# d8ahazard/AudioLab

Hardware: AMD Instinct MI355X
Metric: stems*realtime-factor (44.1kHz stereo) (higher is better)
Workload: dtype bf16; 1 GPU; MDX-Net UVR 4-stem (4x TFC-TDF U-Net L=11 g=48 dim_f=3072 dim_t=256 n_fft=6144), 300 s 44.1 kHz stereo in total, margin chunker, windows/launch=52; stems=4

## Files before the change

audiolab_amd/csrc/tdfnet.hip:

```cpp
#include "mma.h"
#include <alsep_gfx950_asm.h>

#include <map>
#include <type_traits>

namespace {

constexpr int kThreads = 256;

template <typename T> struct Vec16;
template <> struct Vec16<float> { static constexpr int N = 4; };
template <> struct Vec16<bf16_t> { static constexpr int N = 8; };
__device__ __forceinline__ void store_vec(float* p, const float* y) { *reinterpret_cast<float4*>(p) = make_float4(y[0], y[1], y[2], y[3]); }
__device__ __forceinline__ void store_vec(bf16_t* p, const float* y) {
    bf16x8 q;
#pragma unroll
    for (int e = 0; e < 8; ++e) q[e] = (bf16_t)y[e];
    *reinterpret_cast<bf16x8*>(p) = q;
}
__device__ __forceinline__ void load_vec(const float* p, float* x) {
    const float4 q = *reinterpret_cast<const float4*>(p);
    x[0] = q.x; x[1] = q.y; x[2] = q.z; x[3] = q.w;
}
__device__ __forceinline__ void load_vec(const bf16_t* p, float* x) {
// ... 2109 lines not shown
template <int C_, int OCC>
__global__ void __launch_bounds__(kThreads, OCC)
ds_split_stream_kernel(const bf16_t* __restrict__ X, bf16_t* __restrict__ Y, const bf16_t* __restrict__ Wf,
                       const float* __restrict__ scale, const float* __restrict__ shift, int64_t npix, int Tp, int Fp) {
    typedef DsSplitCfg<C_> D;
    const int tid = threadIdx.x, lane = tid & 63, wave = tid >> 6;
    const int l15 = lane & 15, lq = lane >> 4;
    bf16_t* stg = reinterpret_cast<bf16_t*>(alsep_smem);
    bf16x8 wf[D::MTW][D::KS];
#pragma unroll
    for (int j = 0; j < D::MTW; ++j) {
        const int mt = wave + 4 * j;
#pragma unroll
        for (int ks = 0; ks < D::KS; ++ks)
            wf[j][ks] = mt < D::MT ? *reinterpret_cast<const bf16x8*>(Wf + ((size_t)(mt * D::KS + ks) * 64 + lane) * 8) : bf16x8{};
    }
    const int64_t ntile = npix / 64;
    for (int64_t tile = blockIdx.x; tile < ntile; tile += gridDim.x) {
        const int64_t p0 = tile * 64;
        const int64_t fp0 = p0 % Fp, tp = (p0 / Fp) % Tp, bb = p0 / ((int64_t)Fp * Tp);
        const bf16_t* xrow = X + ((bb * 2 * Tp + 2 * tp) * (2 * (int64_t)Fp) + 2 * fp0) * D::C;
        f32x4 acc[D::MTW][4];
#pragma unroll
        for (int j = 0; j < D::MTW; ++j)
#pragma unroll
            for (int ni = 0; ni < 4; ++ni) acc[j][ni] = f32x4{0.f, 0.f, 0.f, 0.f};
#pragma unroll
        for (int ks = 0; ks < D::KS; ++ks) {
            const int k = ks * 32 + lq * 8;
            const int dy = k / (2 * D::C), rem = k % (2 * D::C);
            bf16x8 xf[4];
#pragma unroll
            for (int ni = 0; ni < 4; ++ni)
                xf[ni] = *reinterpret_cast<const bf16x8*>(xrow + (int64_t)dy * (2 * (int64_t)Fp * D::C) + (int64_t)(ni * 16 + l15) * (2 * D::C) + rem);
#pragma unroll
            for (int j = 0; j < D::MTW; ++j)
                if (wave + 4 * j < D::MT) {
#pragma unroll
                    for (int ni = 0; ni < 4; ++ni) mma_step(acc[j][ni], wf[j][ks], xf[ni]);
                }
        }
#pragma unroll
        for (int j = 0; j < D::MTW; ++j) {
            const int mt = wave + 4 * j;
            if (mt < D::MT) {
                const f32x4 scv = *reinterpret_cast<const f32x4*>(scale + mt * 16 + 4 * lq);
                const f32x4 shv = *reinterpret_cast<const f32x4*>(shift + mt * 16 + 4 * lq);
#pragma unroll
                for (int ni = 0; ni < 4; ++ni) {
                    float y[4];
#pragma unroll
                    for (int r = 0; r < 4; ++r) y[r] = fmaxf(fmaf(acc[j][ni][r], scv[r], shv[r]), 0.f);
                    store4(stg + (ni * 16 + l15) * D::MS + mt * 16 + 4 * lq, y);
                }
            }
        }
        __syncthreads();
        bf16_t* yrow = Y + p0 * D::M;
        for (int it = tid; it < 64 * D::M / 8; it += kThreads)
            *reinterpret_cast<vec16*>(yrow + (size_t)it * 8) = lds_read16_align8(stg + (it / (D::M / 8)) * D::MS + (it % (D::M / 8)) * 8);
        __syncthreads();
    }
}

template <int CIN, int C2_, int NI_> struct UsCfg {
    static constexpr int C = CIN, C2 = C2_, NI = NI_, PX = 16 * NI_, MT = C2_ / 16, KS = (CIN + 31) / 32;
    static constexpr int PS = C2_ + 4;
    static constexpr size_t lds_bytes = 2 * (size_t)(2 * PX) * PS * sizeof(float);
    static_assert(C2_ % 16 == 0 && CIN % 8 == 0 && (2 * 2 * PX * (C2_ / 8)) % kThreads == 0, "us stream geometry");
};
template <int CIN, int C2_, int NI_, int OCC = 1>
__global__ void __launch_bounds__(kThreads, OCC)
us_stream_kernel(const bf16_t* __restrict__ X, bf16_t* __restrict__ Y, const bf16_t* __restrict__ Wf,
                 const float* __restrict__ scale, const float* __restrict__ shift, const bf16_t* __restrict__ skip,
                 int64_t npix, int Tp, int Fp) {
    typedef UsCfg<CIN, C2_, NI_> U;
    const int tid = threadIdx.x, lane = tid & 63, wave = tid >> 6;
    const int l15 = lane & 15, lq = lane >> 4;
    const int dy = wave >> 1, dx = wave & 1;
    float* stg = reinterpret_cast<float*>(alsep_smem);
    bf16x8 wf[U::MT][U::KS];
#pragma unroll
    for (int mt = 0; mt < U::MT; ++mt)
#pragma unroll
        for (int ks = 0; ks < U::KS; ++ks)
            wf[mt][ks] = *reinterpret_cast<const bf16x8*>(Wf + ((size_t)((wave * U::MT + mt) * U::KS + ks) * 64 + lane) * 8);
    constexpr bool SS_REGS = U::MT <= 3;
    constexpr int SSN = SS_REGS ? U::MT : 1;
    float sc[SSN][4], sh[SSN][4];
    if (SS_REGS) {
#pragma unroll
        for (int mt = 0; mt < SSN; ++mt)
#pragma unroll
            for (int r = 0; r < 4; ++r) { sc[mt][r] = scale[mt * 16 + 4 * lq + r]; sh[mt][r] = shift[mt * 16 + 4 * lq + r]; }
    }
    const int64_t ntile = npix / U::PX;
    for (int64_t tile = blockIdx.x; tile < ntile; tile += gridDim.x) {
        const int64_t p0 = tile * U::PX;
        const int64_t fp0 = p0 % Fp, tp = (p0 / Fp) % Tp, bb = p0 / ((int64_t)Fp * Tp);
        f32x4 acc[U::MT][U::NI];
#pragma unroll
        for (int mt = 0; mt < U::MT; ++mt)
#pragma unroll
            for (int ni = 0; ni < U::NI; ++ni) acc[mt][ni] = f32x4{0.f, 0.f, 0.f, 0.f};
#pragma unroll
        for (int ks = 0; ks < U::KS; ++ks) {
            bf16x8 xf[U::NI];
#pragma unroll
            for (int ni = 0; ni < U::NI; ++ni) {
                if (U::C % 32 == 0 || ks * 32 + lq * 8 < U::C)
                    xf[ni] = *reinterpret_cast<const bf16x8*>(X + (p0 + ni * 16 + l15) * U::C + ks * 32 + lq * 8);
                else
                    xf[ni] = bf16x8{};
            }
#pragma unroll
            for (int mt = 0; mt < U::MT; ++mt)
#pragma unroll
                for (int ni = 0; ni < U::NI; ++ni) mma_step(acc[mt][ni], wf[mt][ks], xf[ni]);
        }
#pragma unroll
        for (int mt = 0; mt < U::MT; ++mt)
#pragma unroll
            for (int ni = 0; ni < U::NI; ++ni) {
                f32x4 y;
                if (SS_REGS) {
#pragma unroll
                    for (int r = 0; r < 4; ++r) y[r] = fmaxf(fmaf(acc[mt][ni][r], sc[SS_REGS ? mt : 0][r], sh[SS_REGS ? mt : 0][r]), 0.f);
                } else {
                    const f32x4 scv = *reinterpret_cast<const f32x4*>(scale + mt * 16 + 4 * lq);
                    const f32x4 shv = *reinterpret_cast<const f32x4*>(shift + mt * 16 + 4 * lq);
#pragma unroll
                    for (int r = 0; r < 4; ++r) y[r] = fmaxf(fmaf(acc[mt][ni][r], scv[r], shv[r]), 0.f);
                }
                *reinterpret_cast<f32x4*>(stg + ((size_t)dy * (2 * U::PX) + 2 * (ni * 16 + l15) + dx) * U::PS + mt * 16 + 4 * lq) = y;
            }
        __syncthreads();
        constexpr int NG = U::C2 / 8, ROWG = 2 * U::PX * NG;
#pragma unroll
        for (int it = 0; it < 2 * ROWG / kThreads; ++it) {
            const int gidx = it * kThreads + tid;
            const int row = gidx / ROWG, rem = gidx % ROWG;
            const int64_t o = ((bb * 2 * Tp + 2 * tp + row) * (2 * (int64_t)Fp) + 2 * fp0) * U::C2 + (int64_t)rem * 8;
            const float* src = stg + ((size_t)row * (2 * U::PX) + rem / NG) * U::PS + (rem % NG) * 8;
            const f32x4 lo = *reinterpret_cast<const f32x4*>(src);
            const f32x4 hi = *reinterpret_cast<const f32x4*>(src + 4);
            const bf16x8 sk = *reinterpret_cast<const bf16x8*>(skip + o);
            bf16x8 q;
#pragma unroll
            for (int e = 0; e < 4; ++e) { q[e] = (bf16_t)(lo[e] * (float)sk[e]); q[4 + e] = (bf16_t)(hi[e] * (float)sk[4 + e]); }
            stream_store(reinterpret_cast<bf16x8*>(Y + o), q);
        }
        __syncthreads();
    }
}

#ifndef ALSEP_F16_TU
#include "tdfnet_f32s.h"
#endif

struct DevBuf {
    void* p = nullptr;
    size_t bytes = 0;
};

struct ConvLayer {
    DevBuf w, scale, shift;
    DevBuf w_big;
    DevBuf w_mny;
    DevBuf w_mq;
    int cin = 0, cout = 0;
    bool dma_path = false;
    int split = 0;
    unsigned* range_flag = nullptr;
};
struct GemmLayer {
    DevBuf w, bias, scale, shift;
    int M = 0, K = 0, Kp = 0, Mp = 0;
    bool has_bias = false;
    bool split = false;
    unsigned* range_flag = nullptr;
    bool dma_path = false;
    DevBuf wfrag;
    DevBuf wwide;
};
struct Block {
    std::vector<ConvLayer> tfc;
    std::vector<GemmLayer> tdf;
};

}

struct alsep_net {
    alsep_ctx* ctx = nullptr;
    alsep_net_config cfg{};
    int n = 0;
    bool split = false;
    DevBuf range_flag;
    std::vector<DevBuf> owned;
    DevBuf first_w, first_scale, first_shift, final_w, final_b, zero_page;
    std::vector<Block> enc, dec;
    Block bott;
    std::vector<GemmLayer> ds, us;
};

namespace {

typedef std::map<std::string, std::vector<float>> TensorMap;

template <typename T> T host_cast(float v);
template <> float host_cast<float>(float v) { return v; }
template <> bf16_t host_cast<bf16_t>(float v) { return (bf16_t)v; }

int upload(alsep_net* net, const void* src, size_t bytes, DevBuf* out) {
    void* d = nullptr;
    if (hipMalloc(&d, bytes ? bytes : 16) != hipSuccess) return alsep_fail(net->ctx, ALSEP_ERR_NOMEM, "hipMalloc(%zu) failed", bytes);
    out->p = d;
    out->bytes = bytes;
    net->owned.push_back(*out);
    if (bytes) ALSEP_HIP(net->ctx, hipMemcpy(d, src, bytes, hipMemcpyHostToDevice));
    return ALSEP_OK;
}

const std::vector<float>* find(const TensorMap& tm, const std::string& name, int64_t numel, alsep_ctx* ctx, bool required = true) {
    auto it = tm.find(name);
    if (it == tm.end()) {
        if (required) alsep_fail(ctx, ALSEP_ERR_ARG, "missing tensor '%s'", name.c_str());
        return nullptr;
    }
    if ((int64_t)it->second.size() != numel) {
        alsep_fail(ctx, ALSEP_ERR_ARG, "tensor '%s' has %zu elements, expected %lld", name.c_str(), it->second.size(), (long long)numel);
        return nullptr;
    }
    return &it->second;
}

template <typename T> struct ConvSel;
template <> struct ConvSel<bf16_t> { static constexpr int KC = 48, BN = 48; };
template <> struct ConvSel<float> { static constexpr int KC = 16, BN = 48; };
template <typename T> struct ConvSel16;
template <> struct ConvSel16<bf16_t> { static constexpr int KC = 16, BN = 16; };
template <> struct ConvSel16<float> { static constexpr int KC = 16, BN = 16; };

template <typename T> bool conv_uses_main(int cin, int cout) {
    return cin % ConvSel<T>::KC == 0 && cout % ConvSel<T>::BN == 0;
}

template <typename T, int KC, int BN>
std::vector<T> pack_conv3x3(const std::vector<float>& w, int cin, int cout) {
    typedef ConvCfg<T, KC, BN, 64> Cf;
    const int nq = cin / KC, nn = cout / BN;
    std::vector<T> out((size_t)nn * nq * BN * Cf::KP, host_cast<T>(0.f));
    for (int j = 0; j < nn; ++j)
        for (int q = 0; q < nq; ++q)
            for (int r = 0; r < BN; ++r)
                for (int grp = 0; grp < Cf::NG; ++grp)
                    for (int e = 0; e < Cf::G; ++e) {
                        const int tap = grp / Cf::CG, cg = grp % Cf::CG;
                        const int ci = q * KC + cg * Cf::G + e, co = j * BN + r;
                        const float v = w[(((size_t)co * cin + ci) * 3 + tap / 3) * 3 + tap % 3];
                        out[(((size_t)j * nq + q) * BN + r) * Cf::KP + grp * Cf::G + e] = host_cast<T>(v);
                    }
    return out;
}

std::vector<bf16_t> pack_conv3x3_dma(const std::vector<float>& w, int cin, int cout) {
    typedef ConvB16<64> Cf;
    const int nq = cin / Cf::KC, nn = cout / Cf::BN;
    std::vector<bf16_t> out((size_t)nn * nq * Cf::WGROUPS * 8, host_cast<bf16_t>(0.f));
    for (int j = 0; j < nn; ++j)
        for (int q = 0; q < nq; ++q)
            for (int r = 0; r < Cf::BN; ++r)
                for (int grp = 0; grp < Cf::NG; ++grp)
                    for (int e = 0; e < 8; ++e) {
                        const int tap = grp / Cf::CG, cg = grp % Cf::CG;
                        const int ci = q * Cf::KC + cg * 8 + e, co = j * Cf::BN + r;
                        const float v = w[(((size_t)co * cin + ci) * 3 + tap / 3) * 3 + tap % 3];
                        const int pg = grp ^ ((r >> 1) & 7);
                        out[((((size_t)j * nq + q) * Cf::BN + r) * Cf::WG + pg) * 8 + e] = host_cast<bf16_t>(v);
                    }
    return out;
}

template <int NY>
std::vector<bf16_t> pack_conv3x3_big(const std::vector<float>& w, int cin) {
    const int cout = 48 * NY;
    std::vector<float> wp(w.size());
    const size_t row = (size_t)cin * 9;
    for (int R = 0; R < cout; ++R) std::copy(w.begin() + ConvBig<NY>::channel_of_row(R) * row, w.begin() + (ConvBig<NY>::channel_of_row(R) + 1) * row, wp.begin() + R * row);
    return pack_conv3x3_dma(wp, cin, cout);
}

#ifdef ALSEP_EXPERIMENTS
template <int NY>
std::vector<bf16_t> pack_conv3x3_mny(const std::vector<float>& w, int cin) {
    typedef ConvMny<NY> Cf;
    const int nq = cin / Cf::KC;
    std::vector<bf16_t> out((size_t)nq * Cf::PARTS * Cf::WGROUPS * 8, host_cast<bf16_t>(0.f));
    for (int q = 0; q < nq; ++q)
        for (int kt = 0; kt < Cf::PARTS; ++kt)
            for (int R = 0; R < Cf::ROWS; ++R)
                for (int stl = 0; stl < Cf::ksteps_of_part(kt); ++stl)
                    for (int lq = 0; lq < 4; ++lq) {
                        const int grp = 4 * (kt * Cf::KS + stl) + lq;
                        if (grp >= Cf::NG) continue;
                        const int tap = grp / Cf::CG, cg = grp % Cf::CG, co = ConvBig<NY>::channel_of_row(R);
                        const size_t dst = ((((size_t)q * Cf::PARTS + kt) * Cf::ROWS + R) * Cf::WG + 4 * stl + (lq ^ Cf::wswz(R))) * 8;
// ... 597 lines not shown
#endif
#ifdef ALSEP_EXPERIMENTS
    if (defer) {
        ALSEP_HIP(ctx, hipFuncSetAttribute((const void*)conv3x3_bf16_m0_kernel<false, true>, hipFuncAttributeMaxDynamicSharedMemorySize, (int)Cf::lds_bytes));
        hipLaunchKernelGGL((conv3x3_bf16_m0_kernel<false, true>), dim3((unsigned)gx), dim3(kBigThreads), Cf::lds_bytes, ctx->stream, X, Y,
                           (const bf16_t*)L.w_big.p, (const float*)L.scale.p, (const float*)L.shift.p, zero_page, Th, Fw, L.cin, L.cout, tiles_t,
                           tiles_f, (int)ntiles, nullptr);
    } else
#endif
    {
        (void)defer;
        ALSEP_HIP(ctx, hipFuncSetAttribute((const void*)conv3x3_bf16_m0_kernel<false, false>, hipFuncAttributeMaxDynamicSharedMemorySize, (int)Cf::lds_bytes));
        hipLaunchKernelGGL((conv3x3_bf16_m0_kernel<false, false>), dim3((unsigned)gx), dim3(kBigThreads), Cf::lds_bytes, ctx->stream, X, Y,
                           (const bf16_t*)L.w_big.p, (const float*)L.scale.p, (const float*)L.shift.p, zero_page, Th, Fw, L.cin, L.cout, tiles_t,
                           tiles_f, (int)ntiles, nullptr);
    }
    ALSEP_LAUNCH_CHECK(ctx, "conv3x3_bf16_m0_kernel");
    return ALSEP_OK;
}

int conv_m0_enabled() {
    static const int v = [] { const char* e = getenv("ALSEP_CONV_M0"); return e ? atoi(e) : 1; }();
    return v;
}

int conv_mq_enabled() {
    static const int v = [] { const char* e = getenv("ALSEP_CONV_MQ"); return e ? atoi(e) : 1; }();
    return v;
}

#ifdef ALSEP_EXPERIMENTS
int conv_mny_enabled() {
    static const int v = [] { const char* e = getenv("ALSEP_CONV_MNY"); return e ? atoi(e) : 0; }();
    return v;
}
#endif

int conv_big_enabled() {
    static const int v = [] { const char* e = getenv("ALSEP_CONV_BIG"); return e ? atoi(e) : 1; }();
    return v;
}

int conv_big3_enabled() {
    static const int v = [] { const char* e = getenv("ALSEP_CONV_BIG3"); return e ? atoi(e) : 1; }();
    return v;
}

#ifdef ALSEP_EXPERIMENTS
int conv_pipe_enabled() {
    static const int v = [] { const char* e = getenv("ALSEP_CONV_PIPE"); return e ? atoi(e) : 0; }();
    return v;
}
#endif

int conv_regw_enabled() {
    static const int v = [] { const char* e = getenv("ALSEP_CONV_REGW"); return e ? atoi(e) : 1; }();
    return v;
}

int run_conv_dma(alsep_ctx* ctx, const ConvLayer& L, const bf16_t* X, bf16_t* Y, const bf16_t* zp, int64_t B, int Th, int Fw) {
    if (conv_m0_enabled() && L.cin == 48 && L.cout == 48 && Th % 8 == 0 && Fw % 48 == 0 &&
        (conv_m0_enabled() >= 2 || B * (Th / 8) * (Fw / 48) >= 256))
        return launch_conv_m0(ctx, L, X, Y, zp, B, Th, Fw);
    if (conv_regw_enabled() && Th % 4 == 0 && Fw % 64 == 0 && L.cin == L.cout) {
        if (L.cin == 48 && conv_regw_enabled() == 3) return launch_conv_regw<1>(ctx, L, X, Y, zp, B, Th, Fw);
        if (L.cin == 48) return launch_conv_regw<1, 3, 2, 32>(ctx, L, X, Y, zp, B, Th, Fw);
        if (L.cin == 96 && conv_regw_enabled() >= 2) return launch_conv_regw<2>(ctx, L, X, Y, zp, B, Th, Fw);
    }
    if (conv_big_enabled() && Th % 8 == 0 && Fw % 64 == 0 && L.cin == L.cout &&
        (conv_big_enabled() >= 2 || B * (Th / 8) * (Fw / 64) >= 96)) {
        switch (L.cout / 48) {
            case 2:
                if (conv_mq_enabled()) return launch_conv_mq(ctx, L, X, Y, zp, B, Th, Fw);
#ifdef ALSEP_EXPERIMENTS
                if (conv_mny_enabled() & 1) return launch_conv_mny<2>(ctx, L, X, Y, zp, B, Th, Fw);
                return launch_conv_big<2>(ctx, L, X, Y, zp, B, Th, Fw);
#else
                break;
#endif
            case 3:
#ifdef ALSEP_EXPERIMENTS
                if (conv_mny_enabled() & 2) return launch_conv_mny<3>(ctx, L, X, Y, zp, B, Th, Fw);
#endif
                if (conv_big3_enabled()) return launch_conv_big<3>(ctx, L, X, Y, zp, B, Th, Fw);
                break;
            default: break;
        }
    }
#ifdef ALSEP_EXPERIMENTS
    if (conv_pipe_enabled() && Th % 4 == 0 && Fw % 64 == 0 && L.cin == L.cout &&
        (conv_pipe_enabled() >= 2 || B * (Th / 4) * (Fw / 64) >= 128)) {
        switch (L.cout / 48) {
            case 2: return launch_conv_pipe<2>(ctx, L, X, Y, zp, B, Th, Fw);
            case 3: return launch_conv_pipe<3>(ctx, L, X, Y, zp, B, Th, Fw);
            default: break;
        }
    }
#endif
    if (Fw >= 64 && Fw % 64 == 0) return launch_conv_dma<64>(ctx, L, X, Y, zp, B, Th, Fw);
    if (Fw >= 32) return launch_conv_dma<32>(ctx, L, X, Y, zp, B, Th, Fw);
    return launch_conv_dma<16>(ctx, L, X, Y, zp, B, Th, Fw);
}
int run_conv_dma(alsep_ctx* ctx, const ConvLayer&, const float*, float*, const float*, int64_t, int, int) {
    return alsep_fail(ctx, ALSEP_ERR_STATE, "LDS-DMA conv path is bf16 only");
}

#ifndef ALSEP_F16_TU
template <int KC, int BN, int TW>
int launch_conv_split(alsep_ctx* ctx, const ConvLayer& L, const float* X, float* Y, int64_t B, int Th, int Fw) {
    typedef ConvSCfg<KC, BN, TW> Cf;
    const int tiles_t = (int)ceil_div64(Th, Cf::TH), tiles_f = (int)ceil_div64(Fw, TW);
    const int64_t ntiles = B * tiles_t * tiles_f;
    const int nyc = L.cout / BN;
    if (ntiles * nyc > 0x7fffffff) return alsep_fail(ctx, ALSEP_ERR_ARG, "conv3x3: too many tiles");
    ALSEP_HIP(ctx, hipFuncSetAttribute((const void*)conv3x3_f32s_kernel<KC, BN, TW>, hipFuncAttributeMaxDynamicSharedMemorySize,
                                       (int)Cf::lds_bytes));
    ProfScope prof(ctx, TW >= 32 ? ALSEP_PROF_CONV3X3 : ALSEP_PROF_CONV3X3_SMALL);
    prof.work(18.0 * (double)L.cin * L.cout * B * Th * Fw, 4.0 * B * Th * Fw * (L.cin + L.cout));
    const int nyf = (ntiles % 8 == 0 && nyc > 1) ? 1 : 0;
    const dim3 grid = nyf ? dim3((unsigned)(ntiles * nyc)) : dim3((unsigned)ntiles, nyc);
    hipLaunchKernelGGL((conv3x3_f32s_kernel<KC, BN, TW>), grid, dim3(kThreads), Cf::lds_bytes, ctx->stream, X, Y,
                       (const hs_t*)L.w.p, (const float*)L.scale.p, (const float*)L.shift.p, Th, Fw, L.cin, L.cout, tiles_t, tiles_f,
                       (int)ntiles, nyf, L.range_flag);
    ALSEP_LAUNCH_CHECK(ctx, "conv3x3_f32s_kernel");
    return ALSEP_OK;
}
template <int KC, int BN>
int run_conv_split_tw(alsep_ctx* ctx, const ConvLayer& L, const float* X, float* Y, int64_t B, int Th, int Fw) {
    if (Fw >= 32) return launch_conv_split<KC, BN, 32>(ctx, L, X, Y, B, Th, Fw);
    return launch_conv_split<KC, BN, 16>(ctx, L, X, Y, B, Th, Fw);
}
int run_conv_split(alsep_ctx* ctx, const ConvLayer& L, const float* X, float* Y, int64_t B, int Th, int Fw) {
    return L.split == 24 ? run_conv_split_tw<24, 48>(ctx, L, X, Y, B, Th, Fw) : run_conv_split_tw<16, 16>(ctx, L, X, Y, B, Th, Fw);
}
int run_conv_split(alsep_ctx* ctx, const ConvLayer&, const bf16_t*, bf16_t*, int64_t, int, int) {
    return alsep_fail(ctx, ALSEP_ERR_STATE, "split contraction is a float32 mode");
}
#endif

template <typename T>
int run_conv(alsep_ctx* ctx, const ConvLayer& L, const T* X, T* Y, int64_t B, int Th, int Fw, const void* zero_page) {
#ifndef ALSEP_F16_TU
    if (L.split) return run_conv_split(ctx, L, X, Y, B, Th, Fw);
#endif
    if (L.dma_path) return run_conv_dma(ctx, L, X, Y, (const T*)zero_page, B, Th, Fw);
    if (conv_uses_main<T>(L.cin, L.cout)) return run_conv_tw<T, ConvSel<T>::KC, ConvSel<T>::BN>(ctx, L, X, Y, B, Th, Fw);
    return run_conv_tw<T, ConvSel16<T>::KC, ConvSel16<T>::BN>(ctx, L, X, Y, B, Th, Fw);
}

int pix_stream_enabled() {
    static const int v = [] { const char* e = getenv("ALSEP_PIX_STREAM"); return e ? atoi(e) : 1; }();
    return v;
}
int run_pix_stream(alsep_ctx* ctx, int mode, const GemmLayer& L, const bf16_t* X, bf16_t* Y, const bf16_t* skip, int64_t ncols,
                   int Tp, int Fp) {
    ProfScope prof(ctx, ALSEP_PROF_PIX);
    const int64_t ntile = ncols / 64;
    if (mode == PIX_DS && L.M == Ds48::M) {
        const size_t lds = 4 * 64 * Ds48::MS * sizeof(bf16_t);
        const int64_t gx = std::min<int64_t>(ceil_div64(ntile, 4), 256);
        hipLaunchKernelGGL(ds48_stream_kernel, dim3((unsigned)gx), dim3(kThreads), lds, ctx->stream, X, Y, (const bf16_t*)L.wfrag.p,
                           (const float*)L.scale.p, (const float*)L.shift.p, ncols, Tp, Fp);
        note_launch(ctx, "ds48_stream_kernel");
    } else if (mode == PIX_DS && L.M == DsSplitCfg<96>::M) {
        const size_t lds = 64 * DsSplitCfg<96>::MS * sizeof(bf16_t);
        const int64_t gx = std::min<int64_t>(ntile, 512);
        hipLaunchKernelGGL((ds_split_stream_kernel<96, 2>), dim3((unsigned)gx), dim3(kThreads), lds, ctx->stream, X, Y,
                           (const bf16_t*)L.wfrag.p, (const float*)L.scale.p, (const float*)L.shift.p, ncols, Tp, Fp);
        note_launch(ctx, "ds_split_stream_kernel<96>");
    } else if (mode == PIX_DS) {
        const size_t lds = 64 * DsSplitCfg<144>::MS * sizeof(bf16_t);
        const int64_t gx = std::min<int64_t>(ntile, 512);
        hipLaunchKernelGGL((ds_split_stream_kernel<144, 1>), dim3((unsigned)gx), dim3(kThreads), lds, ctx->stream, X, Y,
                           (const bf16_t*)L.wfrag.p, (const float*)L.scale.p, (const float*)L.shift.p, ncols, Tp, Fp);
        note_launch(ctx, "ds_split_stream_kernel<144>");
    } else {
#define ALSEP_US(CIN_, C2_, NI_, OCC_, GX_)                                                                                 \
    {                                                                                                                       \
        typedef UsCfg<CIN_, C2_, NI_> U;                                                                                    \
        ALSEP_HIP(ctx, hipFuncSetAttribute((const void*)us_stream_kernel<CIN_, C2_, NI_, OCC_>,                             \
                                           hipFuncAttributeMaxDynamicSharedMemorySize, (int)U::lds_bytes));                 \
        const int64_t gx = std::min<int64_t>(ncols / U::PX, GX_);                                                           \
        hipLaunchKernelGGL((us_stream_kernel<CIN_, C2_, NI_, OCC_>), dim3((unsigned)gx), dim3(kThreads), U::lds_bytes,      \
                           ctx->stream, X, Y, (const bf16_t*)L.wfrag.p, (const float*)L.scale.p, (const float*)L.shift.p,   \
                           skip, ncols, Tp, Fp);                                                                            \
        note_launch(ctx, "us_stream_kernel<" #CIN_ "," #C2_ ">");                                                          \
    }
        if (L.K == 96) ALSEP_US(96, 48, 4, 1, 512)
        else if (L.K == 144) ALSEP_US(144, 96, 2, 2, 512)
        else ALSEP_US(192, 144, 2, 1, 256)
#undef ALSEP_US
    }
    note_launch(ctx, mode == PIX_DS ? "ds_stream_kernel" : "us_stream_kernel");
    ALSEP_LAUNCH_CHECK(ctx, "pix stream kernel");
    return ALSEP_OK;
}
int run_pix_stream(alsep_ctx* ctx, int, const GemmLayer&, const float*, float*, const float*, int64_t, int, int) {
    return alsep_fail(ctx, ALSEP_ERR_STATE, "streaming ds/us path is bf16 only");
}

#ifndef ALSEP_F16_TU
template <int MODE>
int run_pix_split(alsep_ctx* ctx, const GemmLayer& L, const float* X, float* Y, const float* skip, int64_t ncols, int Tp, int Fp, int C, int C2) {
    typedef GemmSCfg Gc;
    const int64_t gx = ceil_div64(ncols, Gc::BC);
    if (gx > 0x7fffffff) return alsep_fail(ctx, ALSEP_ERR_ARG, "pix_gemm: too many column tiles");
    ALSEP_HIP(ctx, hipFuncSetAttribute((const void*)pix_gemm_f32s_kernel<MODE>, hipFuncAttributeMaxDynamicSharedMemorySize, (int)Gc::lds_bytes));
    ProfScope prof(ctx, ALSEP_PROF_PIX);
    const int nrb = L.Mp / Gc::BR;
    const int fast = (nrb > 1 && gx % 8 == 0 && gx * nrb <= 0x7fffffff) ? nrb : 0;
    hipLaunchKernelGGL((pix_gemm_f32s_kernel<MODE>), fast ? dim3((unsigned)(gx * nrb)) : dim3((unsigned)gx, nrb), dim3(kThreads), Gc::lds_bytes,
                       ctx->stream, X, Y, (const hs_t*)L.w.p, (const float*)L.scale.p, (const float*)L.shift.p, skip, L.M, L.Mp, L.K, L.Kp, ncols,
                       Tp, Fp, C, C2, L.range_flag, fast);
    ALSEP_LAUNCH_CHECK(ctx, "pix_gemm_f32s_kernel");
    return ALSEP_OK;
}
template <int MODE>
int run_pix_split(alsep_ctx* ctx, const GemmLayer&, const bf16_t*, bf16_t*, const bf16_t*, int64_t, int, int, int, int) {
    return alsep_fail(ctx, ALSEP_ERR_STATE, "split contraction is a float32 mode");
}
int run_tdf_split(alsep_ctx* ctx, const GemmLayer& L, const float* X, float* Y, const float* R, int64_t BT, int C) {
    typedef GemmSCfg Gc;
    const int64_t nunits = BT * (C / 16);
    const int64_t gx = ceil_div64(nunits, 8);
    if (gx > 0x7fffffff) return alsep_fail(ctx, ALSEP_ERR_ARG, "tdf_gemm: too many column tiles");
    const float* bias = L.has_bias ? (const float*)L.bias.p : nullptr;
    ProfScope prof(ctx, ALSEP_PROF_TDF);
    const int nrb = L.Mp / Gc::BR;
    const int fast = (nrb > 1 && gx % 8 == 0 && gx * nrb <= 0x7fffffff) ? nrb : 0;
    const dim3 grid = fast ? dim3((unsigned)(gx * nrb)) : dim3((unsigned)gx, nrb);
    if (R) {
        ALSEP_HIP(ctx, hipFuncSetAttribute((const void*)tdf_gemm_f32s_kernel<true>, hipFuncAttributeMaxDynamicSharedMemorySize, (int)Gc::lds_bytes));
        hipLaunchKernelGGL((tdf_gemm_f32s_kernel<true>), grid, dim3(kThreads), Gc::lds_bytes, ctx->stream, X, Y, (const hs_t*)L.w.p, bias,
                           (const float*)L.scale.p, (const float*)L.shift.p, R, L.M, L.Mp, L.K, L.Kp, nunits, C, L.range_flag, fast);
    } else {
        ALSEP_HIP(ctx, hipFuncSetAttribute((const void*)tdf_gemm_f32s_kernel<false>, hipFuncAttributeMaxDynamicSharedMemorySize, (int)Gc::lds_bytes));
        hipLaunchKernelGGL((tdf_gemm_f32s_kernel<false>), grid, dim3(kThreads), Gc::lds_bytes, ctx->stream, X, Y, (const hs_t*)L.w.p, bias,
                           (const float*)L.scale.p, (const float*)L.shift.p, R, L.M, L.Mp, L.K, L.Kp, nunits, C, L.range_flag, fast);
    }
    ALSEP_LAUNCH_CHECK(ctx, "tdf_gemm_f32s_kernel");
    return ALSEP_OK;
}
int run_tdf_split(alsep_ctx* ctx, const GemmLayer&, const bf16_t*, bf16_t*, const bf16_t*, int64_t, int) {
    return alsep_fail(ctx, ALSEP_ERR_STATE, "split contraction is a float32 mode");
}
#endif

template <typename T, int MODE>
int run_pix(alsep_ctx* ctx, const GemmLayer& L, const T* X, T* Y, const T* skip, int64_t ncols, int Tp, int Fp, int C, int C2) {
    typedef GemmCfg<T> Gc;
#ifndef ALSEP_F16_TU
    if (L.split) return run_pix_split<MODE>(ctx, L, X, Y, skip, ncols, Tp, Fp, C, C2);
#endif
    if (L.wfrag.p && pix_stream_enabled() && Fp % 64 == 0) return run_pix_stream(ctx, MODE, L, X, Y, skip, ncols, Tp, Fp);
    const int64_t gx = ceil_div64(ncols, Gc::BC);
    if (gx > 0x7fffffff) return alsep_fail(ctx, ALSEP_ERR_ARG, "pix_gemm: too many column tiles");
    ProfScope prof(ctx, ALSEP_PROF_PIX);
    hipLaunchKernelGGL((pix_gemm_kernel<T, MODE>), dim3((unsigned)gx, L.Mp / Gc::BR), dim3(kThreads), Gc::lds_bytes,
                       ctx->stream, X, Y, (const T*)L.w.p, (const float*)L.scale.p, (const float*)L.shift.p, skip,
                       L.M, L.K, L.Kp, ncols, Tp, Fp, C, C2);
    ALSEP_LAUNCH_CHECK(ctx, "pix_gemm_kernel");
    return ALSEP_OK;
}

int tdf_wide_mode() {
    static const int v = [] { const char* e = getenv("ALSEP_TDF_WIDE"); return e ? atoi(e) : 1; }();
    return v;
}
struct FinalFold {
    const float* w;
    const float* b;
    void* out;
    float alpha;
    bool done;
};
int tdf_final_mode() {
    static const int v = [] { const char* e = getenv("ALSEP_TDF_FINAL"); return e ? atoi(e) : 1; }();
    return v;
}
enum { kTdfPersistK384 = 1, kTdfPersistK192 = 2, kTdfPersistFinal = 4 };
constexpr int kTdfPersistRouted = kTdfPersistK384 | kTdfPersistK192 | kTdfPersistFinal;
int tdf_persist_mode() {
    static const int v = [] { const char* e = getenv("ALSEP_TDF_PERSIST"); return e ? atoi(e) : 1; }();
    return v;
}
template <int NT, bool FINAL>
void launch_tdf_persist_inst(alsep_ctx* ctx, hipError_t& attr, unsigned grid, const GemmLayer& L, const bf16_t* X, bf16_t* Y,
                             const bf16_t* R, int64_t nitems, int C, const FinalFold* fin) {
    constexpr int lds = (int)TdfPersist::lds_bytes(NT, FINAL);
    attr = hipFuncSetAttribute((const void*)tdf_bf16_persist_kernel<NT, FINAL>, hipFuncAttributeMaxDynamicSharedMemorySize, lds);
    if (attr != hipSuccess) return;
    hipLaunchKernelGGL((tdf_bf16_persist_kernel<NT, FINAL>), dim3(grid), dim3(TdfPersist::THREADS), lds, ctx->stream, X, Y,
                       (const bf16_t*)L.wwide.p, L.has_bias ? (const float*)L.bias.p : nullptr, (const float*)L.scale.p,
                       (const float*)L.shift.p, R, L.M, nitems, C, fin ? fin->w : nullptr, fin ? fin->b : nullptr,
                       fin ? (bf16_t*)fin->out : nullptr, fin ? fin->alpha : 0.f);
}
int launch_tdf_persist(alsep_ctx* ctx, const GemmLayer& L, const bf16_t* X, bf16_t* Y, const bf16_t* R, int64_t nunits, int C,
                       FinalFold* fin) {
    static const int cap = [] { const char* e = getenv("ALSEP_TDF_PERSIST_GRID"); return e ? atoi(e) : 0; }();
    const int64_t nitems = nunits / TdfPersist::UN;
    int64_t grid = device_cu_count(ctx);
    if (cap > 0 && cap < grid) grid = cap;
    if (nitems < grid) grid = nitems;
    hipError_t attr = hipSuccess;
    if (fin && L.K == 384) launch_tdf_persist_inst<6, true>(ctx, attr, (unsigned)grid, L, X, Y, R, nitems, C, fin);
    else if (fin) launch_tdf_persist_inst<3, true>(ctx, attr, (unsigned)grid, L, X, Y, R, nitems, C, fin);
    else if (L.K == 384) launch_tdf_persist_inst<6, false>(ctx, attr, (unsigned)grid, L, X, Y, R, nitems, C, nullptr);
    else launch_tdf_persist_inst<3, false>(ctx, attr, (unsigned)grid, L, X, Y, R, nitems, C, nullptr);
    ALSEP_HIP(ctx, attr);
    if (fin) {
        fin->done = true;
// ... 351 lines not shown
```

Measured before the change: 5998 stems*x_realtime.

## Add persistent multi-stage pipelined kernels for downsample and upsample pixel GEMMs

Adds persistent ds_pipe and us_pipe kernels. Each launches one block per CU and streams its tiles through an LDS ring using async global-to-LDS loads with vmcnt-gated prefetch depth, double-buffered fragment reads and output staging through LDS. By default these replace the existing stream kernels for the ds96, ds144, us192 and us144 layers. The aim is to overlap memory traffic with MFMA work and to keep weights resident in registers across tiles. The trade-off is fixed LDS footprints of up to 160 KB, one block per CU, and new hand-written asm LDS paths that carry correctness risk.

```diff
diff --git a/audiolab_amd/csrc/tdfnet.hip b/audiolab_amd/csrc/tdfnet.hip
--- a/audiolab_amd/csrc/tdfnet.hip
+++ b/audiolab_amd/csrc/tdfnet.hip
@@ -2285,6 +2285,347 @@
         }
         __syncthreads();
     }
+}
+
+#ifdef ALSEP_CPU_EMUL
+static inline void lds_write_async_b64(bf16_t* lds_ptr, const bf16x4& v) { std::memcpy(lds_ptr, &v, 8); }
+template <int OFF>
+static inline void lds_read_async_f32x4(f32x4& dst, const float* lds_ptr) { std::memcpy(&dst, reinterpret_cast<const char*>(lds_ptr) + OFF, 16); }
+#else
+template <int OFF>
+__device__ __forceinline__ void lds_read_async_f32x4(f32x4& dst, const float* lds_ptr) {
+    static_assert(OFF >= 0 && OFF < 65536 && OFF % 16 == 0, "ds offset field");
+    const unsigned addr = (unsigned)(unsigned long long)(__attribute__((address_space(3))) const void*)lds_ptr;
+    asm volatile("ds_read_b128 %0, %1 offset:%2" : "=v"(dst) : "v"(addr), "n"(OFF) : "memory");
+}
+__device__ __forceinline__ void lds_write_async_b64(bf16_t* lds_ptr, const bf16x4& v) {
+    const unsigned addr = (unsigned)(unsigned long long)(__attribute__((address_space(3))) void*)lds_ptr;
+    asm volatile("ds_write_b64 %0, %1" : : "v"(addr), "v"(v) : "memory");
+}
+#endif
+template <typename F, int... I>
+__device__ __forceinline__ void static_for_impl(F&& f, std::integer_sequence<int, I...>) {
+    (f(std::integral_constant<int, I>{}), ...);
+}
+template <int N, typename F>
+__device__ __forceinline__ void static_for(F&& f) {
+    static_for_impl(f, std::make_integer_sequence<int, N>{});
+}
+template <int D, int ND, int NS>
+__device__ __forceinline__ void pipe_wait_tile(int i, int n) {
+    static_assert(D >= 1 && D * NS + (D - 1) * ND < 64, "vmcnt is a 6-bit counter");
+    if (i + D - 1 < n) {
+        if (i > D) wait_vmcnt<D * NS + (D - 1) * ND>();
+        else wait_vmcnt<(D - 1) * ND>();
+    } else {
+        wait_vmcnt<0>();
+    }
+}
+
+template <int C_, int PX_, int D_> struct DsPipeCfg {
+    typedef DsSplitCfg<C_> S;
+    static constexpr int C = C_, M = S::M, MT = S::MT, KS = S::KS, MTW = S::MTW, PX = PX_, NI = PX_ / 16, D = D_, NSLOT = D_ + 1;
+    static constexpr int SR = C_ / 4, HALF_G = PX * SR, TILE_G = 2 * HALF_G, ND = TILE_G / kThreads;
+    static constexpr int MS = M + 8, OUT_GW = PX * M / 8 / 4, NS = (OUT_GW + 63) / 64;
+    static constexpr size_t tile_bytes = (size_t)TILE_G * 16, img_bytes = (size_t)PX * MS * sizeof(bf16_t);
+    static constexpr size_t lds_bytes = NSLOT * tile_bytes + 2 * img_bytes;
+    __host__ __device__ static constexpr int swz(int row) { return SR % 8 == 0 ? (row & 7) : ((row >> 2) & 2); }
+    static_assert(PX % 16 == 0 && HALF_G % 64 == 0 && TILE_G % kThreads == 0 && KS % 2 == 0 && SR % 4 == 0 && (PX * M / 8) % 4 == 0,
+                  "ds pipe geometry");
+    static_assert(lds_bytes <= 160 * 1024 && tile_bytes < 65536, "LDS of a CU; ds offset field");
+};
+template <int C_, int PX_, int D_>
+__global__ void __launch_bounds__(kThreads, 1)
+ds_pipe_kernel(const bf16_t* __restrict__ X, bf16_t* __restrict__ Y, const bf16_t* __restrict__ Wf,
+               const float* __restrict__ scale, const float* __restrict__ shift, int64_t npix, int Tp, int Fp) {
+    typedef DsPipeCfg<C_, PX_, D_> P;
+    const int tid = threadIdx.x, lane = tid & 63;
+    const int wave = __builtin_amdgcn_readfirstlane(tid >> 6);
+    const int l15 = lane & 15, lq = lane >> 4;
+    char* ring = alsep_smem;
+    bf16_t* img = reinterpret_cast<bf16_t*>(alsep_smem + P::NSLOT * P::tile_bytes);
+    bf16x8 wf[P::MTW][P::KS];
+    f32x4 sc[P::MTW], sh[P::MTW];
+#pragma unroll
+    for (int j = 0; j < P::MTW; ++j) {
+        const int mt = wave + 4 * j;
+#pragma unroll
+        for (int ks = 0; ks < P::KS; ++ks)
+            wf[j][ks] = mt < P::MT ? *reinterpret_cast<const bf16x8*>(Wf + ((size_t)(mt * P::KS + ks) * 64 + lane) * 8) : bf16x8{};
+        sc[j] = mt < P::MT ? *reinterpret_cast<const f32x4*>(scale + mt * 16 + 4 * lq) : f32x4{0.f, 0.f, 0.f, 0.f};
+        sh[j] = mt < P::MT ? *reinterpret_cast<const f32x4*>(shift + mt * 16 + 4 * lq) : f32x4{0.f, 0.f, 0.f, 0.f};
+    }
+    unsigned xoff[P::ND];
+#pragma unroll
+    for (int q = 0; q < P::ND; ++q) {
+        const int pg = (wave * P::ND + q) * 64 + lane;
+        const int dy = pg / P::HALF_G, row = (pg % P::HALF_G) / P::SR, gp = pg % P::SR;
+        xoff[q] = (unsigned)dy * (2u * (unsigned)Fp * P::C * (unsigned)sizeof(bf16_t)) + (unsigned)((row * P::SR + (gp ^ P::swz(row))) * 16);
+    }
+    unsigned bk[P::KS / 2];
+#pragma unroll
+    for (int kk = 0; kk < P::KS / 2; ++kk) bk[kk] = (unsigned)((l15 * P::SR + ((kk * 4 + lq) ^ P::swz(l15))) * 16);
+    unsigned ioff[P::NS];
+#pragma unroll
+    for (int t = 0; t < P::NS; ++t) {
+        const int g = wave * P::OUT_GW + t * 64 + lane;
+        ioff[t] = (unsigned)(((g / (P::M / 8)) * P::MS + (g % (P::M / 8)) * 8) * (int)sizeof(bf16_t));
+    }
+
+    const int64_t ntile = npix / P::PX;
+    const int nmy = (int)((ntile - (int64_t)blockIdx.x + gridDim.x - 1) / gridDim.x);
+    auto issue = [&](int j) {
+        const int64_t p0 = ((int64_t)blockIdx.x + (int64_t)j * gridDim.x) * P::PX;
+        const int64_t fp0 = p0 % Fp, tp = (p0 / Fp) % Tp, bb = p0 / ((int64_t)Fp * Tp);
+        const ALSEP_GLOBAL char* src = opaque_uniform_gptr(
+            reinterpret_cast<const char*>(X + ((bb * 2 * Tp + 2 * tp) * (2 * (int64_t)Fp) + 2 * fp0) * P::C));
+        char* dst = ring + (size_t)(j % P::NSLOT) * P::tile_bytes + (size_t)wave * (P::ND * 1024);
+#pragma unroll
+        for (int q = 0; q < P::ND; ++q) glds16_base(src, xoff[q], dst + q * 1024);
+    };
+    auto copy_out = [&](int j) {
+        const int64_t p0 = ((int64_t)blockIdx.x + (int64_t)j * gridDim.x) * P::PX;
+        ALSEP_GLOBAL char* yb = const_cast<ALSEP_GLOBAL char*>(
+            opaque_uniform_gptr(reinterpret_cast<const char*>(Y + p0 * P::M + (int64_t)wave * (P::OUT_GW * 8))));
+        const char* im = reinterpret_cast<const char*>(img) + (size_t)(j & 1) * P::img_bytes;
+        bf16x8 q[P::NS];
+#pragma unroll
+        for (int t = 0; t < P::NS; ++t)
+            if (t * 64 + lane < P::OUT_GW) lds_read_async_b128<0>(q[t], reinterpret_cast<const bf16_t*>(im + ioff[t]));
+        lds_wait_n<0>();
+#pragma unroll
+        for (int t = 0; t < P::NS; ++t)
+            if (t * 64 + lane < P::OUT_GW) stream_store(reinterpret_cast<ALSEP_GLOBAL bf16x8*>(yb + (unsigned)(t * 64 + lane) * 16u), q[t]);
+    };
+
+    wait_vmcnt<0>();
+#pragma unroll
+    for (int j = 0; j < P::D; ++j)
+        if (j < nmy) issue(j);
+    for (int i = 0; i < nmy; ++i) {
+        pipe_wait_tile<P::D, P::ND, P::NS>(i, nmy);
+        barrier_nodrain();
+        if (i + P::D < nmy) issue(i + P::D);
+        if (i > 0) copy_out(i - 1);
+        const bf16_t* slot = reinterpret_cast<const bf16_t*>(ring + (size_t)(i % P::NSLOT) * P::tile_bytes);
+        f32x4 acc[P::MTW][P::NI];
+#pragma unroll
+        for (int j = 0; j < P::MTW; ++j)
+#pragma unroll
+            for (int ni = 0; ni < P::NI; ++ni) acc[j][ni] = f32x4{0.f, 0.f, 0.f, 0.f};
+        bf16x8 xf[2][P::NI];
+        static_for<P::NI>([&](auto nic) {
+            constexpr int ni = decltype(nic)::value;
+            lds_read_async_b128<ni * 16 * P::SR * 16>(xf[0][ni], slot + bk[0] / sizeof(bf16_t));
+        });
+        static_for<P::KS>([&](auto ksc) {
+            constexpr int ks = decltype(ksc)::value, b = ks & 1;
+            if constexpr (ks + 1 < P::KS) {
+                constexpr int dy1 = (ks + 1) / (P::KS / 2), kk1 = (ks + 1) % (P::KS / 2);
+                static_for<P::NI>([&](auto nic) {
+                    constexpr int ni = decltype(nic)::value;
+                    lds_read_async_b128<dy1 * P::HALF_G * 16 + ni * 16 * P::SR * 16>(xf[1 - b][ni], slot + bk[kk1] / sizeof(bf16_t));
+                });
+                lds_wait_n<P::NI>();
+            } else {
+                lds_wait_n<0>();
+            }
+#pragma unroll
+            for (int j = 0; j < P::MTW; ++j)
+                if (wave + 4 * j < P::MT) {
+#pragma unroll
+                    for (int ni = 0; ni < P::NI; ++ni) mma_step(acc[j][ni], wf[j][ks], xf[b][ni]);
+                }
+        });
+        bf16_t* im = img + (size_t)(i & 1) * (P::PX * P::MS);
+#pragma unroll
+        for (int j = 0; j < P::MTW; ++j) {
+            const int mt = wave + 4 * j;
+            if (mt < P::MT) {
+#pragma unroll
+                for (int ni = 0; ni < P::NI; ++ni) {
+                    bf16x4 q;
+#pragma unroll
+                    for (int r = 0; r < 4; ++r) q[r] = (bf16_t)fmaxf(fmaf(acc[j][ni][r], sc[j][r], sh[j][r]), 0.f);
+                    lds_write_async_b64(im + (ni * 16 + l15) * P::MS + mt * 16 + 4 * lq, q);
+                }
+            }
+        }
+    }
+    barrier_nodrain();
+    copy_out(nmy - 1);
+}
+
+template <int CIN, int C2_, int NI_, int D_> struct UsPipeCfg {
+    typedef UsCfg<CIN, C2_, NI_> U;
+    static constexpr int C = CIN, C2 = C2_, NI = NI_, PX = 16 * NI_, MT = U::MT, KS = U::KS, D = D_, NSX = D_ + 1, NSS = D_ + 2;
+    static constexpr int SRX = CIN / 8, XW_G = (PX / 4) * SRX, NDX = (XW_G + 63) / 64, XREG = NDX * 1024;
+    static constexpr int NG = C2_ / 8, ROW_G = 2 * PX * NG, S_G = 2 * ROW_G, NDS = S_G / kThreads;
+    static constexpr int ND = NDX + NDS, NS = NDS;
+    static constexpr size_t x_bytes = 4 * (size_t)XREG, s_bytes = (size_t)S_G * 16, bn_bytes = 2 * (size_t)C2_ * sizeof(float);
+    static constexpr size_t lds_bytes = NSX * x_bytes + NSS * s_bytes + bn_bytes;
+    __host__ __device__ static constexpr int swz(int row) { return SRX % 8 == 0 ? (row & 7) : 0; }
+    __host__ __device__ static constexpr int rot(int px) { return NG % 4 == 0 ? ((px >> 2) & 7) : ((px >> 3) & 3); }
+    static_assert(PX % 32 == 0 && ROW_G % 64 == 0 && S_G % kThreads == 0 && (NG % 4 == 0 ? NG >= 8 : NG >= 4), "us pipe geometry");
+    static_assert(lds_bytes <= 160 * 1024 && x_bytes < 65536 && s_bytes < 65536, "LDS of a CU; ds offset field");
+};
+template <int CIN, int C2_, int NI_, int D_>
+__global__ void __launch_bounds__(kThreads, 1)
+us_pipe_kernel(const bf16_t* __restrict__ X, bf16_t* __restrict__ Y, const bf16_t* __restrict__ Wf,
+               const float* __restrict__ scale, const float* __restrict__ shift, const bf16_t* __restrict__ skip,
+               int64_t npix, int Tp, int Fp) {
+    typedef UsPipeCfg<CIN, C2_, NI_, D_> P;
+    const int tid = threadIdx.x, lane = tid & 63;
+    const int wave = __builtin_amdgcn_readfirstlane(tid >> 6);
+    const int l15 = lane & 15, lq = lane >> 4;
+    const int dy = wave >> 1, dx = wave & 1;
+    char* xring = alsep_smem;
+    char* sring = alsep_smem + P::NSX * P::x_bytes;
+    float* bn = reinterpret_cast<float*>(alsep_smem + P::NSX * P::x_bytes + P::NSS * P::s_bytes);
+    bf16x8 wf[P::MT][P::KS];
+#pragma unroll
+    for (int mt = 0; mt < P::MT; ++mt)
+#pragma unroll
+        for (int ks = 0; ks < P::KS; ++ks)
+            wf[mt][ks] = *reinterpret_cast<const bf16x8*>(Wf + ((size_t)((wave * P::MT + mt) * P::KS + ks) * 64 + lane) * 8);
+    for (int c = tid; c < 2 * P::C2; c += kThreads) bn[c] = c < P::C2 ? scale[c] : shift[c - P::C2];
+    unsigned xoff[P::NDX], soff[P::NDS];
+#pragma unroll
+    for (int q = 0; q < P::NDX; ++q) {
+        const int gi = q * 64 + lane < P::XW_G ? q * 64 + lane : P::XW_G - 1;
+        const int row = gi / P::SRX, gp = gi % P::SRX;
+        xoff[q] = (unsigned)(((wave * (P::PX / 4) + row) * P::SRX + (gp ^ P::swz(row))) * 16);
+    }
+#pragma unroll
+    for (int q = 0; q < P::NDS; ++q) {
+        const int pg = (wave * P::NDS + q) * 64 + lane;
+        const int row = pg / P::ROW_G, px = (pg % P::ROW_G) / P::NG, gp = pg % P::NG;
+        soff[q] = (unsigned)row * (2u * (unsigned)Fp * P::C2 * (unsigned)sizeof(bf16_t)) + (unsigned)((px * P::NG + (gp - P::rot(px) + P::NG) % P::NG) * 16);
+    }
+    unsigned bk[P::KS];
+#pragma unroll
+    for (int ks = 0; ks < P::KS; ++ks) {
+        const int g = ks * 4 + lq < P::SRX ? ks * 4 + lq : P::SRX - 1;
+        bk[ks] = (unsigned)((l15 >> 3) * P::XREG + ((l15 & 7) * P::SRX + (g ^ P::swz(l15 & 7))) * 16);
+    }
+    const bool klast_ok = P::C % 32 == 0 || (P::KS - 1) * 4 + lq < P::SRX;
+    const int opx = 2 * l15 + dx;
+    const unsigned ebase = (unsigned)((dy * P::ROW_G + opx * P::NG) * 16);
+    const int erot = (lq >> 1) + P::rot(opx);
+
+    const int64_t ntile = npix / P::PX;
+    const int nmy = (int)((ntile - (int64_t)blockIdx.x + gridDim.x - 1) / gridDim.x);
+    auto out_base = [&](int j) {
+        const int64_t p0 = ((int64_t)blockIdx.x + (int64_t)j * gridDim.x) * P::PX;
+        const int64_t fp0 = p0 % Fp, tp = (p0 / Fp) % Tp, bb = p0 / ((int64_t)Fp * Tp);
+        return ((bb * 2 * Tp + 2 * tp) * (2 * (int64_t)Fp) + 2 * fp0) * P::C2;
+    };
+    auto issue = [&](int j) {
+        const int64_t p0 = ((int64_t)blockIdx.x + (int64_t)j * gridDim.x) * P::PX;
+        const ALSEP_GLOBAL char* xs = opaque_uniform_gptr(reinterpret_cast<const char*>(X + p0 * P::C));
+        const ALSEP_GLOBAL char* ss = opaque_uniform_gptr(reinterpret_cast<const char*>(skip + out_base(j)));
+        char* xd = xring + (size_t)(j % P::NSX) * P::x_bytes + (size_t)wave * P::XREG;
+        char* sd = sring + (size_t)(j % P::NSS) * P::s_bytes + (size_t)wave * (P::NDS * 1024);
+#pragma unroll
+        for (int q = 0; q < P::NDX; ++q) glds16_base(xs, xoff[q], xd + q * 1024);
+#pragma unroll
+        for (int q = 0; q < P::NDS; ++q) glds16_base(ss, soff[q], sd + q * 1024);
+    };
+    auto copy_out = [&](int j) {
+        ALSEP_GLOBAL char* yb = const_cast<ALSEP_GLOBAL char*>(opaque_uniform_gptr(reinterpret_cast<const char*>(Y + out_base(j))));
+        const bf16_t* sd = reinterpret_cast<const bf16_t*>(sring + (size_t)(j % P::NSS) * P::s_bytes + (size_t)wave * (P::NDS * 1024)) + lane * 8;
+        bf16x8 q[P::NDS];
+        static_for<P::NDS>([&](auto tc) {
+            constexpr int t = decltype(tc)::value;
+            lds_read_async_b128<t * 1024>(q[t], sd);
+        });
+        lds_wait_n<0>();
+#pragma unroll
+        for (int t = 0; t < P::NDS; ++t) stream_store(reinterpret_cast<ALSEP_GLOBAL bf16x8*>(yb + soff[t]), q[t]);
+    };
+
+    wait_vmcnt<0>();
+#pragma unroll
+    for (int j = 0; j < P::D; ++j)
+        if (j < nmy) issue(j);
+    for (int i = 0; i < nmy; ++i) {
+        pipe_wait_tile<P::D, P::ND, P::NS>(i, nmy);
+        barrier_nodrain();
+        if (i + P::D < nmy) issue(i + P::D);
+        if (i > 0) copy_out(i - 1);
+        const bf16_t* xs = reinterpret_cast<const bf16_t*>(xring + (size_t)(i % P::NSX) * P::x_bytes);
+        f32x4 acc[P::MT][P::NI];
+#pragma unroll
+        for (int mt = 0; mt < P::MT; ++mt)
+#pragma unroll
+            for (int ni = 0; ni < P::NI; ++ni) acc[mt][ni] = f32x4{0.f, 0.f, 0.f, 0.f};
+        bf16x8 xf[2][P::NI];
+        static_for<P::NI>([&](auto nic) {
+            constexpr int ni = decltype(nic)::value;
+            lds_read_async_b128<ni * 2 * P::XREG>(xf[0][ni], xs + bk[0] / sizeof(bf16_t));
+        });
+        static_for<P::KS>([&](auto ksc) {
+            constexpr int ks = decltype(ksc)::value, b = ks & 1;
+            if constexpr (ks + 1 < P::KS) {
+                static_for<P::NI>([&](auto nic) {
+                    constexpr int ni = decltype(nic)::value;
+                    lds_read_async_b128<ni * 2 * P::XREG>(xf[1 - b][ni], xs + bk[ks + 1] / sizeof(bf16_t));
+                });
+                lds_wait_n<P::NI>();
+            } else {
+                lds_wait_n<0>();
+                if (P::C % 32 != 0) {
+#pragma unroll
+                    for (int ni = 0; ni < P::NI; ++ni) xf[b][ni] = klast_ok ? xf[b][ni] : bf16x8{};
+                }
+            }
+#pragma unroll
+            for (int mt = 0; mt < P::MT; ++mt)
+#pragma unroll
+                for (int ni = 0; ni < P::NI; ++ni) mma_step(acc[mt][ni], wf[mt][ks], xf[b][ni]);
+        });
+        bf16_t* sl = reinterpret_cast<bf16_t*>(sring + (size_t)(i % P::NSS) * P::s_bytes + ebase);
+        const float* bnl = bn + 4 * lq;
+        auto eoff = [&](int mt) {
+            int t = 2 * mt + erot;
+            t = t >= P::NG ? t - P::NG : t;
+            return t * 8;
+        };
+        bf16x8 ev[2][P::NI];
+        f32x4 scv[2], shv[2];
+        auto eread = [&](auto mtc) {
+            constexpr int mt = decltype(mtc)::value, eb = mt & 1;
+            const bf16_t* p = sl + eoff(mt);
+            static_for<P::NI>([&](auto nic) {
+                constexpr int ni = decltype(nic)::value;
+                lds_read_async_b128<ni * 32 * P::NG * 16>(ev[eb][ni], p);
+            });
+            lds_read_async_f32x4<0>(scv[eb], bnl + mt * 16);
+            lds_read_async_f32x4<P::C2 * 4>(shv[eb], bnl + mt * 16);
+        };
+        eread(std::integral_constant<int, 0>{});
+        static_for<P::MT>([&](auto mtc) {
+            constexpr int mt = decltype(mtc)::value, b = mt & 1;
+            if constexpr (mt + 1 < P::MT) {
+                eread(std::integral_constant<int, mt + 1>{});
+                lds_wait_n<P::NI + 2>();
+            } else {
+                lds_wait_n<0>();
+            }
+            bf16_t* p = sl + eoff(mt) + (lq & 1) * 4;
+            static_for<P::NI>([&](auto nic) {
+                constexpr int ni = decltype(nic)::value;
+                const bf16x4 sk = (lq & 1) ? __builtin_shufflevector(ev[b][ni], ev[b][ni], 4, 5, 6, 7)
+                                           : __builtin_shufflevector(ev[b][ni], ev[b][ni], 0, 1, 2, 3);
+                bf16x4 q;
+#pragma unroll
+                for (int r = 0; r < 4; ++r) q[r] = (bf16_t)(fmaxf(fmaf(acc[mt][ni][r], scv[b][r], shv[b][r]), 0.f) * (float)sk[r]);
+                lds_write_async_b64(p + ni * 32 * P::NG * 8, q);
+            });
+        });
+    }
+    barrier_nodrain();
+    copy_out(nmy - 1);
 }
 
 #ifndef ALSEP_F16_TU
@@ -3188,11 +3529,57 @@
     static const int v = [] { const char* e = getenv("ALSEP_PIX_STREAM"); return e ? atoi(e) : 1; }();
     return v;
 }
+enum { kPixPipeDs96 = 1, kPixPipeDs144 = 2, kPixPipeUs192 = 4, kPixPipeUs144 = 8 };
+constexpr int kPixPipeRouted = kPixPipeDs96 | kPixPipeDs144 | kPixPipeUs192 | kPixPipeUs144;
+bool pix_pipe_routed(int kind) {
+    static const int v = [] { const char* e = getenv("ALSEP_PIX_PIPE"); return e ? atoi(e) : 1; }();
+    return v >= 2 || (v == 1 && (kPixPipeRouted & kind));
+}
+unsigned pix_pipe_grid(alsep_ctx* ctx, int64_t ntile) {
+    static const int cap = [] { const char* e = getenv("ALSEP_PIX_PIPE_GRID"); return e ? atoi(e) : 0; }();
+    int64_t grid = device_cu_count(ctx);
+    if (cap > 0 && cap < grid) grid = cap;
+    return (unsigned)std::min<int64_t>(grid, ntile);
+}
+template <int C_, int PX_, int D_>
+hipError_t launch_ds_pipe(alsep_ctx* ctx, const GemmLayer& L, const bf16_t* X, bf16_t* Y, int64_t ncols, int Tp, int Fp) {
+    typedef DsPipeCfg<C_, PX_, D_> P;
+    const hipError_t e = hipFuncSetAttribute((const void*)ds_pipe_kernel<C_, PX_, D_>, hipFuncAttributeMaxDynamicSharedMemorySize, (int)P::lds_bytes);
+    if (e != hipSuccess) return e;
+    hipLaunchKernelGGL((ds_pipe_kernel<C_, PX_, D_>), dim3(pix_pipe_grid(ctx, ncols / P::PX)), dim3(kThreads), P::lds_bytes, ctx->stream, X, Y,
+                       (const bf16_t*)L.wfrag.p, (const float*)L.scale.p, (const float*)L.shift.p, ncols, Tp, Fp);
+    return hipSuccess;
+}
+template <int CIN, int C2_, int NI_, int D_>
+hipError_t launch_us_pipe(alsep_ctx* ctx, const GemmLayer& L, const bf16_t* X, bf16_t* Y, const bf16_t* skip, int64_t ncols, int Tp, int Fp) {
+    typedef UsPipeCfg<CIN, C2_, NI_, D_> P;
+    const hipError_t e = hipFuncSetAttribute((const void*)us_pipe_kernel<CIN, C2_, NI_, D_>, hipFuncAttributeMaxDynamicSharedMemorySize, (int)P::lds_bytes);
+    if (e != hipSuccess) return e;
+    hipLaunchKernelGGL((us_pipe_kernel<CIN, C2_, NI_, D_>), dim3(pix_pipe_grid(ctx, ncols / P::PX)), dim3(kThreads), P::lds_bytes, ctx->stream, X, Y,
+                       (const bf16_t*)L.wfrag.p, (const float*)L.scale.p, (const float*)L.shift.p, skip, ncols, Tp, Fp);
+    return hipSuccess;
+}
 int run_pix_stream(alsep_ctx* ctx, int mode, const GemmLayer& L, const bf16_t* X, bf16_t* Y, const bf16_t* skip, int64_t ncols,
                    int Tp, int Fp) {
     ProfScope prof(ctx, ALSEP_PROF_PIX);
     const int64_t ntile = ncols / 64;
-    if (mode == PIX_DS && L.M == Ds48::M) {
+    if (mode == PIX_DS && L.M == DsSplitCfg<96>::M && pix_pipe_routed(kPixPipeDs96)) {
+        ALSEP_HIP(ctx, (launch_ds_pipe<96, 64, 1>(ctx, L, X, Y, ncols, Tp, Fp)));
+        note_launch(ctx, "ds_pipe_kernel<96>");
+        note_launch(ctx, "ds_split_stream_kernel<96>");
+    } else if (mode == PIX_DS && L.M == DsSplitCfg<144>::M && pix_pipe_routed(kPixPipeDs144)) {
+        ALSEP_HIP(ctx, (launch_ds_pipe<144, 32, 2>(ctx, L, X, Y, ncols, Tp, Fp)));
+        note_launch(ctx, "ds_pipe_kernel<144>");
+        note_launch(ctx, "ds_split_stream_kernel<144>");
+    } else if (mode != PIX_DS && L.K == 192 && pix_pipe_routed(kPixPipeUs192)) {
+        ALSEP_HIP(ctx, (launch_us_pipe<192, 144, 2, 1>(ctx, L, X, Y, skip, ncols, Tp, Fp)));
+        note_launch(ctx, "us_pipe_kernel<192,144>");
+        note_launch(ctx, "us_stream_kernel<192,144>");
+    } else if (mode != PIX_DS && L.K == 144 && pix_pipe_routed(kPixPipeUs144)) {
+        ALSEP_HIP(ctx, (launch_us_pipe<144, 96, 2, 2>(ctx, L, X, Y, skip, ncols, Tp, Fp)));
+        note_launch(ctx, "us_pipe_kernel<144,96>");
+        note_launch(ctx, "us_stream_kernel<144,96>");
+    } else if (mode == PIX_DS && L.M == Ds48::M) {
         const size_t lds = 4 * 64 * Ds48::MS * sizeof(bf16_t);
         const int64_t gx = std::min<int64_t>(ceil_div64(ntile, 4), 256);
         hipLaunchKernelGGL(ds48_stream_kernel, dim3((unsigned)gx), dim3(kThreads), lds, ctx->stream, X, Y, (const bf16_t*)L.wfrag.p,
```

Measured after the change: 6183 stems*x_realtime, median of 6. +3.1%, better.
